# DerekGloudemans/3D-playground

Hardware: AMD Instinct MI355X
Metric: training images/sec at 1920x1080, ResNet-50 3D-RetinaNet (higher is better)
Workload: dtype f32; 1 GPU; resnet50 directional 3D-RetinaNet, 1920x1080 synthetic frames, batch 8 per GPU, 10 GT boxes/image, fp32, fwd+loss+bwd+clip+Adam (BASELINE configs[1]); global_batch=8, parallelism=dp1

## Files before the change

3d-playground_amd/csrc/conv_wino.hip:

```cpp
#include "common.h"
#include "mfma_split.h"

__device__ __forceinline__ float4 f4(float s) { return make_float4(s, s, s, s); }
typedef float nt_f4 __attribute__((ext_vector_type(4)));
__device__ __forceinline__ float4 ld_stream(const float *p) {
    const nt_f4 v = __builtin_nontemporal_load(reinterpret_cast<const nt_f4 *>(p));
    return make_float4(v.x, v.y, v.z, v.w);
}
__device__ __forceinline__ void st_stream(float *p, float4 v) { *reinterpret_cast<float4 *>(p) = v; }
__device__ __forceinline__ float4 operator+(float4 a, float4 b) { return make_float4(a.x + b.x, a.y + b.y, a.z + b.z, a.w + b.w); }
__device__ __forceinline__ float4 operator-(float4 a, float4 b) { return make_float4(a.x - b.x, a.y - b.y, a.z - b.z, a.w - b.w); }
__device__ __forceinline__ float4 operator*(float s, float4 a) { return make_float4(s * a.x, s * a.y, s * a.z, s * a.w); }

__device__ __forceinline__ void bt6(const float4 d[6], float4 o[6]) {
    o[0] = 4.f * d[0] - 5.f * d[2] + d[4];
    o[1] = d[3] + d[4] - 4.f * (d[1] + d[2]);
    o[2] = 4.f * (d[1] - d[2]) - d[3] + d[4];
    o[3] = 2.f * (d[3] - d[1]) - d[2] + d[4];
    o[4] = 2.f * (d[1] - d[3]) - d[2] + d[4];
    o[5] = 4.f * d[1] - 5.f * d[3] + d[5];
}
__device__ __forceinline__ void at6(const float4 m[6], float4 o[4]) {
    const float4 s12 = m[1] + m[2], d12 = m[1] - m[2], s34 = m[3] + m[4], d34 = m[3] - m[4];
    o[0] = m[0] + s12 + s34;
    o[1] = d12 + 2.f * d34;
    o[2] = s12 + 4.f * s34;
    o[3] = d12 + 8.f * d34 + m[5];
}


struct WinoProblem { int N, H, W, TH, TW; };
struct WinoTable {
    int n;
    int64_t tile_end[RN_MAX_GROUP];
    WinoProblem p[RN_MAX_GROUP];
    const float *src[RN_MAX_GROUP];
    float *dst[RN_MAX_GROUP];
    const float *add[RN_MAX_GROUP];
    const float *mask[RN_MAX_GROUP];
    unsigned *sign[RN_MAX_GROUP];
    unsigned *amax[RN_MAX_GROUP];
};

#define WINO_GAIN_BT 7
#define WINO_GAIN_A 8
__device__ __forceinline__ void wino_tensor_word(const WinoTable &g, unsigned *tensor_amax, int gain) {
    if (tensor_amax == nullptr || blockIdx.x != 0 || threadIdx.x >= 64) return;
    int e = 0;
#pragma unroll
    for (int i = 0; i < RN_MAX_GROUP; ++i)
        if (i < g.n && g.amax[i] != nullptr) { const int ei = rn_amax_exp_all(g.amax[i], g.p[i].N); e = ei > e ? ei : e; }
    if (threadIdx.x == 0) atomicMax(tensor_amax, rn_amax_word_of_exp(e, gain));
}
__device__ __forceinline__ int wino_locate(const WinoTable &g, int64_t gt, int64_t &local) {
    int q = 0;
#pragma unroll
    for (int i = 0; i < RN_MAX_GROUP - 1; ++i) q += (i + 1 < g.n && gt >= g.tile_end[i]) ? 1 : 0;
    int64_t first = 0;
#pragma unroll
    for (int i = 1; i < RN_MAX_GROUP; ++i)
        if (q == i) first = g.tile_end[i - 1];
    local = gt - first;
    return q;
}

#define WINO_SELECT(q, g, pr, EXTRA)                          \
    WinoProblem pr = g.p[0];                                   \
    _Pragma("unroll") for (int i_ = 1; i_ < RN_MAX_GROUP; ++i_) \
        if (q == i_) { pr = g.p[i_]; EXTRA }

__global__ __launch_bounds__(256) void wino_in_kernel(const WinoTable g, float *__restrict__ V, int C, int64_t t0, int64_t Tpad,
                                                      unsigned *__restrict__ row_amax, unsigned *__restrict__ tensor_amax) {
    wino_tensor_word(g, tensor_amax, WINO_GAIN_BT);
    const int cq = C >> 2;
    const int64_t id = (int64_t)xcd_remap(blockIdx.x, gridDim.x) * 256 + threadIdx.x;
    const int64_t gt_raw = id / cq, t_last = g.tile_end[g.n - 1];
    const int64_t gt = gt_raw < t_last ? gt_raw : t_last - 1;
    const int c4 = (int)(id - gt_raw * cq) * 4;
    int64_t tile;
    const int q = wino_locate(g, gt, tile);
    const float *x = g.src[0];
    const unsigned *xw = g.amax[0];
    WINO_SELECT(q, g, pr, x = g.src[i_]; xw = g.amax[i_];)
    const int H = pr.H, W = pr.W, TW = pr.TW;
    const int n = (int)(tile / (pr.TH * TW));
    const int r = (int)(tile - (int64_t)n * pr.TH * TW);
    const int th = r / TW, tw = r - th * TW;
    const int h0 = 4 * th - 1, w0 = 4 * tw - 1;
    const float *xb = x + (int64_t)n * H * W * C + c4;
    if (row_amax != nullptr) {
        const int e_img = rn_amax_exp_lanes(xw != nullptr ? reinterpret_cast<const unsigned char *>(xw) + (int64_t)n * RN_AMAX_BYTES : nullptr);
        if (gt_raw < t_last && c4 == 0) row_amax[t0 + gt] = rn_amax_word_of_exp(e_img, WINO_GAIN_BT);
    }
    if (gt_raw >= t_last) return;
    float4 t[6][6];
#pragma unroll
    for (int j = 0; j < 6; ++j) {
        float4 d[6], o[6];
        const int w = w0 + j;
#pragma unroll
        for (int i = 0; i < 6; ++i) {
            const int h = h0 + i;
#ifdef RN_WINO_ABL
            const bool ok = (unsigned)h < (unsigned)H && (unsigned)w < (unsigned)W && i >= 1 && i <= 4 && j >= 1 && j <= 4;
#else
            const bool ok = (unsigned)h < (unsigned)H && (unsigned)w < (unsigned)W;
#endif
            d[i] = ok ? *reinterpret_cast<const float4 *>(xb + ((int64_t)h * W + w) * C) : f4(0.f);
        }
        bt6(d, o);
#pragma unroll
        for (int i = 0; i < 6; ++i) t[i][j] = o[i];
    }
    float *vb = V + (t0 + gt) * C + c4;
#pragma unroll
    for (int i = 0; i < 6; ++i) {
        float4 o[6];
        bt6(t[i], o);
#pragma unroll
        for (int j = 0; j < 6; ++j) st_stream(vb + (int64_t)(i * 6 + j) * Tpad * C, o[j]);
    }
}

template <bool PBITS, bool PADD>
__global__ __launch_bounds__(256, 2) void wino_out_kernel(const WinoTable g, const float *__restrict__ M, int Cout, int64_t t0,
                                                       int64_t Tpad, const float *__restrict__ scale,
                                                       const float *__restrict__ shift, int mask_mode, int act, int64_t y_bs) {
    const int cq = Cout >> 2;
    const int64_t id = (int64_t)blockIdx.x * 256 + threadIdx.x;
    const int64_t gt = id / cq;
    float am = 0.f;
    unsigned *yam = nullptr;
    int n_img = 0;
    bool live = false;
    do {
    if (gt >= g.tile_end[g.n - 1]) break;
    live = true;
    const int c4 = (int)(id - gt * cq) * 4;
    int64_t tile;
    const int q = wino_locate(g, gt, tile);
    float *y = g.dst[0];
    const float *add = g.add[0], *mask = g.mask[0];
    unsigned *sign = g.sign[0];
    yam = g.amax[0];
    WINO_SELECT(q, g, pr, y = g.dst[i_]; add = g.add[i_]; mask = g.mask[i_]; sign = g.sign[i_]; yam = g.amax[i_];)
    n_img = (int)(tile / (pr.TH * pr.TW));
    const bool mbits = (mask_mode & RN_MASK_BITS) != 0;
    mask_mode &= 3;
    const int H = pr.H, W = pr.W, TW = pr.TW;
    const int n = (int)(tile / (pr.TH * TW));
    const int r = (int)(tile - (int64_t)n * pr.TH * TW);
    const int th = r / TW, tw = r - th * TW;
    const float *mb = M + (t0 + gt) * Cout + c4;
    float4 t[4][6];
#pragma unroll
    for (int j = 0; j < 6; ++j) {
        float4 m[6], o[4];
#pragma unroll
        for (int i = 0; i < 6; ++i) m[i] = ld_stream(mb + (int64_t)(i * 6 + j) * Tpad * Cout);
        at6(m, o);
#pragma unroll
        for (int i = 0; i < 4; ++i) t[i][j] = o[i];
    }
    float4 sc = f4(1.f), sh = f4(0.f);
    if (scale) sc = *reinterpret_cast<const float4 *>(scale + c4);
    if (shift) sh = *reinterpret_cast<const float4 *>(shift + c4);
    const int64_t ybs = y_bs ? y_bs : (int64_t)H * W * Cout;
#pragma unroll
    for (int i = 0; i < 4; ++i) {
        float4 o[4];
        at6(t[i], o);
        const int oh = 4 * th + i;
        if (oh >= H) break;
        unsigned mkw[4];
        float4 adv[4];
        if constexpr (PBITS || PADD) {
#pragma unroll
            for (int j = 0; j < 4; ++j) {
                const int owc = 4 * tw + j < W ? 4 * tw + j : W - 1;
                const int64_t off = (((int64_t)n * H + oh) * W + owc) * Cout + c4;
                if constexpr (PBITS) mkw[j] = reinterpret_cast<const unsigned *>(mask)[off >> 5] >> ((unsigned)off & 28u);
                if constexpr (PADD) adv[j] = *reinterpret_cast<const float4 *>(add + off);
            }
        }
#pragma unroll
        for (int j = 0; j < 4; ++j) {
            const int ow = 4 * tw + j;
            if (ow >= W) break;
            const int64_t off = (((int64_t)n * H + oh) * W + ow) * Cout + c4;
            const int64_t yoff = (int64_t)n * ybs + ((int64_t)oh * W + ow) * Cout + c4;
            float v[4] = {sc.x * o[j].x + sh.x, sc.y * o[j].y + sh.y, sc.z * o[j].z + sh.z, sc.w * o[j].w + sh.w};
            float mk[4] = {1.f, 1.f, 1.f, 1.f}, ad[4] = {0.f, 0.f, 0.f, 0.f};
            if constexpr (PBITS) {
                const unsigned nb = mkw[j];
                mk[0] = (nb & 1u) ? 1.f : 0.f; mk[1] = (nb & 2u) ? 1.f : 0.f; mk[2] = (nb & 4u) ? 1.f : 0.f; mk[3] = (nb & 8u) ? 1.f : 0.f;
            } else if (mask_mode != 0) { const float4 q4 = rn_mask_load4(mask, off, mbits); mk[0] = q4.x; mk[1] = q4.y; mk[2] = q4.z; mk[3] = q4.w; }
            if constexpr (PADD) { const float4 q4 = adv[j]; ad[0] = q4.x; ad[1] = q4.y; ad[2] = q4.z; ad[3] = q4.w; }
            else if (add) { const float4 q4 = *reinterpret_cast<const float4 *>(add + off); ad[0] = q4.x; ad[1] = q4.y; ad[2] = q4.z; ad[3] = q4.w; }
#pragma unroll
            for (int k = 0; k < 4; ++k) {
                float u = v[k];
                if (mask_mode == 1) u = mk[k] > 0.f ? u : 0.f;
                u += ad[k];
                if (act == 1) u = fmaxf(u, 0.f);
                else if (act == 2) u = 1.0f / (1.0f + expf(-u));
                if (mask_mode == 2) u = mk[k] > 0.f ? u : 0.f;
                v[k] = u;
            }
            *reinterpret_cast<float4 *>(y + yoff) = make_float4(v[0], v[1], v[2], v[3]);
            if (sign != nullptr) rn_sign_store(sign, off, v[0], v[1], v[2], v[3]);
            am = fmaxf(fmaxf(am, fmaxf(fabsf(v[0]), fabsf(v[1]))), fmaxf(fabsf(v[2]), fabsf(v[3])));
        }
    }
    } while (0);
    if (live) rn_amax_note(yam, n_img, am);
}

__global__ void wino_weight_kernel(const float *__restrict__ w, float *__restrict__ U, int Cout, int Cin, int mode,
                                   const float *__restrict__ scale, int rows, int Kpad) {
    const int64_t id = (int64_t)blockIdx.x * 256 + threadIdx.x;
    if (id >= (int64_t)rows * Kpad) return;
    const int row = (int)(id / Kpad), k = (int)(id - (int64_t)row * Kpad);
    const int kdim = mode == 0 ? Cin : Cout;
    float g[3][3];
#pragma unroll
    for (int r = 0; r < 3; ++r)
#pragma unroll
        for (int s = 0; s < 3; ++s) {
            float v = 0.f;
            if (k < kdim) {
                if (mode == 0) v = w[(((int64_t)row * Cin + k) * 3 + r) * 3 + s];
                else v = w[(((int64_t)k * Cin + row) * 3 + (2 - r)) * 3 + (2 - s)] * (scale ? scale[k] : 1.f);
            }
            g[r][s] = v;
        }
    float t[6][3];
#pragma unroll
    for (int s = 0; s < 3; ++s) {
        const float a = g[0][s], b = g[1][s], c = g[2][s];
        t[0][s] = a * (1.f / 4.f);
        t[1][s] = -(a + b + c) * (1.f / 6.f);
        t[2][s] = (b - a - c) * (1.f / 6.f);
        t[3][s] = a * (1.f / 24.f) + b * (1.f / 12.f) + c * (1.f / 6.f);
        t[4][s] = a * (1.f / 24.f) - b * (1.f / 12.f) + c * (1.f / 6.f);
        t[5][s] = c;
    }
#pragma unroll
    for (int i = 0; i < 6; ++i) {
        const float a = t[i][0], b = t[i][1], c = t[i][2];
        const float o[6] = {a * (1.f / 4.f), -(a + b + c) * (1.f / 6.f), (b - a - c) * (1.f / 6.f),
                            a * (1.f / 24.f) + b * (1.f / 12.f) + c * (1.f / 6.f),
                            a * (1.f / 24.f) - b * (1.f / 12.f) + c * (1.f / 6.f), c};
#pragma unroll
        for (int j = 0; j < 6; ++j) U[((int64_t)(i * 6 + j) * rows + row) * Kpad + k] = o[j];
    }
}

__device__ __forceinline__ void a6(const float4 v[4], float4 o[6]) {
    const float4 s02 = v[0] + v[2], s13 = v[1] + v[3];
    o[0] = v[0];
    o[1] = s02 + s13;
    o[2] = s02 - s13;
    const float4 e = v[0] + 4.f * v[2], f = 2.f * v[1] + 8.f * v[3];
    o[3] = e + f;
    o[4] = e - f;
    o[5] = v[3];
}

__global__ __launch_bounds__(256) void wino_dy_kernel(const WinoTable g, float *__restrict__ Z, int C, int64_t t0, int64_t Tpad,
                                                      unsigned *__restrict__ tensor_amax) {
    wino_tensor_word(g, tensor_amax, WINO_GAIN_A);
    const int cq = C >> 2;
    const int64_t id = (int64_t)blockIdx.x * 256 + threadIdx.x;
    const int64_t gt = id / cq;
    if (gt >= g.tile_end[g.n - 1]) return;
    const int c4 = (int)(id - gt * cq) * 4;
    int64_t tile;
    const int q = wino_locate(g, gt, tile);
    const float *dy = g.src[0];
    WINO_SELECT(q, g, pr, dy = g.src[i_];)
    const int H = pr.H, W = pr.W, TW = pr.TW;
    const int n = (int)(tile / (pr.TH * TW));
    const int r = (int)(tile - (int64_t)n * pr.TH * TW);
    const int th = r / TW, tw = r - th * TW;
    const float *yb = dy + (int64_t)n * H * W * C + c4;
    float4 t[6][4];
#pragma unroll
    for (int j = 0; j < 4; ++j) {
        float4 v[4], o[6];
        const int w = 4 * tw + j;
#pragma unroll
        for (int i = 0; i < 4; ++i) {
            const int h = 4 * th + i;
            v[i] = (h < H && w < W) ? *reinterpret_cast<const float4 *>(yb + ((int64_t)h * W + w) * C) : f4(0.f);
        }
        a6(v, o);
#pragma unroll
        for (int a = 0; a < 6; ++a) t[a][j] = o[a];
    }
    float *zb = Z + (t0 + gt) * C + c4;
#pragma unroll
    for (int a = 0; a < 6; ++a) {
        float4 o[6];
        a6(t[a], o);
#pragma unroll
        for (int b = 0; b < 6; ++b) st_stream(zb + (int64_t)(a * 6 + b) * Tpad * C, o[b]);
    }
}

__global__ __launch_bounds__(256) void wino_in_both_kernel(const WinoTable g, float *__restrict__ V, float *__restrict__ Z, int C,
                                                           int64_t t0, int64_t Tpad, unsigned *__restrict__ v_row_amax,
                                                           unsigned *__restrict__ z_tensor_amax) {
    wino_tensor_word(g, z_tensor_amax, WINO_GAIN_A);
    const int cq = C >> 2;
    const int64_t id = (int64_t)xcd_remap(blockIdx.x, gridDim.x) * 256 + threadIdx.x;
    const int64_t gt_raw = id / cq, t_last = g.tile_end[g.n - 1];
    const int64_t gt = gt_raw < t_last ? gt_raw : t_last - 1;
    const int c4 = (int)(id - gt_raw * cq) * 4;
    int64_t tile;
    const int q = wino_locate(g, gt, tile);
    const float *x = g.src[0];
    const unsigned *xw = g.amax[0];
    WINO_SELECT(q, g, pr, x = g.src[i_]; xw = g.amax[i_];)
    const int H = pr.H, W = pr.W, TW = pr.TW;
    const int n = (int)(tile / (pr.TH * TW));
    const int r = (int)(tile - (int64_t)n * pr.TH * TW);
    const int th = r / TW, tw = r - th * TW;
    const int h0 = 4 * th - 1, w0 = 4 * tw - 1;
    const float *xb = x + (int64_t)n * H * W * C + c4;
    if (v_row_amax != nullptr) {
        const int e_img = rn_amax_exp_lanes(xw != nullptr ? reinterpret_cast<const unsigned char *>(xw) + (int64_t)n * RN_AMAX_BYTES : nullptr);
        if (gt_raw < t_last && c4 == 0) v_row_amax[t0 + gt] = rn_amax_word_of_exp(e_img, WINO_GAIN_BT);
    }
    if (gt_raw >= t_last) return;
    float4 t[6][6];
    float4 tz[6][4];
#pragma unroll
    for (int j = 0; j < 6; ++j) {
        float4 d[6], o[6];
        const int w = w0 + j;
#pragma unroll
        for (int i = 0; i < 6; ++i) {
            const int h = h0 + i;
            const bool ok = (unsigned)h < (unsigned)H && (unsigned)w < (unsigned)W;
            d[i] = ok ? *reinterpret_cast<const float4 *>(xb + ((int64_t)h * W + w) * C) : f4(0.f);
        }
        bt6(d, o);
#pragma unroll
        for (int i = 0; i < 6; ++i) t[i][j] = o[i];
        if (j >= 1 && j <= 4) {
            float4 oz[6];
            a6(d + 1, oz);
#pragma unroll
            for (int a = 0; a < 6; ++a) tz[a][j - 1] = oz[a];
        }
    }
    float *zb = Z + (t0 + gt) * C + c4;
#pragma unroll
    for (int a = 0; a < 6; ++a) {
        float4 o[6];
        a6(tz[a], o);
#pragma unroll
        for (int b = 0; b < 6; ++b) st_stream(zb + (int64_t)(a * 6 + b) * Tpad * C, o[b]);
    }
    float *vb = V + (t0 + gt) * C + c4;
#pragma unroll
    for (int i = 0; i < 6; ++i) {
        float4 o[6];
        bt6(t[i], o);
#pragma unroll
        for (int j = 0; j < 6; ++j) st_stream(vb + (int64_t)(i * 6 + j) * Tpad * C, o[j]);
    }
}

__global__ void wino_dw_kernel(const float *__restrict__ dU, float *__restrict__ dw, int Cout, int Cin, int Ku, int Kpad) {
    const int64_t id = (int64_t)blockIdx.x * 256 + threadIdx.x;
    if (id >= (int64_t)Cout * Cin) return;
    const int co = (int)(id / Cin), ci = (int)(id - (int64_t)co * Cin);
    const float *u = dU + (int64_t)co * Ku + ci;
    const int64_t ps = (int64_t)Cout * Ku;
    float t[3][6];
#pragma unroll
    for (int j = 0; j < 6; ++j) {
        float v[6];
#pragma unroll
        for (int i = 0; i < 6; ++i) v[i] = u[(i * 6 + j) * ps];
        t[0][j] = v[0] * (1.f / 4.f) - (v[1] + v[2]) * (1.f / 6.f) + (v[3] + v[4]) * (1.f / 24.f);
        t[1][j] = (v[2] - v[1]) * (1.f / 6.f) + (v[3] - v[4]) * (1.f / 12.f);
        t[2][j] = (v[3] + v[4] - v[1] - v[2]) * (1.f / 6.f) + v[5];
    }
    float *o = dw + (int64_t)co * Kpad + ci;
#pragma unroll
    for (int r = 0; r < 3; ++r) {
        const float *v = t[r];
        o[(r * 3 + 0) * Cin] += v[0] * (1.f / 4.f) - (v[1] + v[2]) * (1.f / 6.f) + (v[3] + v[4]) * (1.f / 24.f);
        o[(r * 3 + 1) * Cin] += (v[2] - v[1]) * (1.f / 6.f) + (v[3] - v[4]) * (1.f / 12.f);
        o[(r * 3 + 2) * Cin] += (v[3] + v[4] - v[1] - v[2]) * (1.f / 6.f) + v[5];
    }
}

static int wino_table(const rn_wino_group *g, WinoTable &t) {
    if (!g || g->n < 1 || g->n > RN_MAX_GROUP) return RN_EINVAL;
    t.n = g->n;
    int64_t end = 0;
    for (int i = 0; i < RN_MAX_GROUP; ++i) {
        const int k = i < g->n ? i : g->n - 1;
        if (g->N[k] <= 0 || g->H[k] <= 0 || g->W[k] <= 0) return RN_EINVAL;
        t.p[i].N = g->N[k]; t.p[i].H = g->H[k]; t.p[i].W = g->W[k];
        t.p[i].TH = (g->H[k] + 3) / 4; t.p[i].TW = (g->W[k] + 3) / 4;
        if (i < g->n) end += (int64_t)g->N[k] * t.p[i].TH * t.p[i].TW;
        t.tile_end[i] = end;
        t.src[i] = g->src[k]; t.dst[i] = g->dst[k]; t.add[i] = g->add[k]; t.mask[i] = g->mask[k];
        t.sign[i] = reinterpret_cast<unsigned *>(g->sign[k]);
        t.amax[i] = reinterpret_cast<unsigned *>(g->amax[k]);
    }
    return RN_OK;
}

extern "C" int rn_wino_input_group(const rn_wino_group *g, float *V, int C, int64_t tile_offset, int64_t Tpad, int dy_form,
                                   void *row_amax, void *tensor_amax, void *stream) {
    WinoTable t;
    const int rc = wino_table(g, t);
    if (rc) return rc;
    if (C <= 0 || (C & 3) || tile_offset < 0 || tile_offset + t.tile_end[t.n - 1] > Tpad) return RN_EINVAL;
    for (int i = 0; i < t.n; ++i)
        if (!t.src[i]) return RN_EINVAL;
    const dim3 grid(rn_blocks(t.tile_end[t.n - 1] * (C >> 2), 256));
    if (dy_form && row_amax != nullptr) return RN_EINVAL;
    if (dy_form) hipLaunchKernelGGL(wino_dy_kernel, grid, dim3(256), 0, (hipStream_t)stream, t, V, C, tile_offset, Tpad,
                                    reinterpret_cast<unsigned *>(tensor_amax));
    else hipLaunchKernelGGL(wino_in_kernel, grid, dim3(256), 0, (hipStream_t)stream, t, V, C, tile_offset, Tpad,
                            reinterpret_cast<unsigned *>(row_amax), reinterpret_cast<unsigned *>(tensor_amax));
    RN_LAUNCH_CHECK();
    return RN_OK;
}

extern "C" int rn_wino_input_both_group(const rn_wino_group *g, float *V, float *Z, int C, int64_t tile_offset, int64_t Tpad,
                                        void *v_row_amax, void *z_tensor_amax, void *stream) {
    WinoTable t;
    const int rc = wino_table(g, t);
    if (rc) return rc;
    if (!V || !Z || C <= 0 || (C & 3) || tile_offset < 0 || tile_offset + t.tile_end[t.n - 1] > Tpad) return RN_EINVAL;
    for (int i = 0; i < t.n; ++i)
        if (!t.src[i]) return RN_EINVAL;
    hipLaunchKernelGGL(wino_in_both_kernel, dim3(rn_blocks(t.tile_end[t.n - 1] * (C >> 2), 256)), dim3(256), 0, (hipStream_t)stream, t,
                       V, Z, C, tile_offset, Tpad, reinterpret_cast<unsigned *>(v_row_amax), reinterpret_cast<unsigned *>(z_tensor_amax));
    RN_LAUNCH_CHECK();
    return RN_OK;
}

extern "C" int rn_wino_output_group(const rn_wino_group *g, const float *M, int Cout, int64_t tile_offset, int64_t Tpad,
                                    const float *scale, const float *shift, int mask_mode, int act, int64_t y_batch_stride,
                                    void *stream) {
    WinoTable t;
    const int rc = wino_table(g, t);
    if (rc) return rc;
    if (Cout <= 0 || (Cout & 3) || tile_offset < 0 || tile_offset + t.tile_end[t.n - 1] > Tpad) return RN_EINVAL;
    if (mask_mode < 0 || (mask_mode & ~(3 | RN_MASK_BITS)) || (mask_mode & 3) == 3 || mask_mode == RN_MASK_BITS) return RN_EINVAL;
    if (act < 0 || act > 2 || y_batch_stride < 0 || (y_batch_stride & 3)) return RN_EINVAL;
    for (int i = 0; i < t.n; ++i) {
        if (!t.dst[i] || (mask_mode != 0) != (t.mask[i] != nullptr)) return RN_EINVAL;
        if (((mask_mode & RN_MASK_BITS) || t.sign[i]) && (Cout & 31)) return RN_EINVAL;
        if (y_batch_stride && y_batch_stride < (int64_t)t.p[i].H * t.p[i].W * Cout) return RN_EINVAL;
    }
    const bool pbits = (mask_mode & RN_MASK_BITS) != 0;
    bool padd = true;
    for (int i = 0; i < t.n; ++i) padd = padd && t.add[i] != nullptr;
    const dim3 grid(rn_blocks(t.tile_end[t.n - 1] * (Cout >> 2), 256));
#define RN_WINO_OUT(B, A) hipLaunchKernelGGL((wino_out_kernel<B, A>), grid, dim3(256), 0, (hipStream_t)stream, t, M, Cout, tile_offset, Tpad, \
                                             scale, shift, mask_mode, act, y_batch_stride)
    if (pbits && padd) RN_WINO_OUT(true, true);
    else if (pbits) RN_WINO_OUT(true, false);
    else if (padd) RN_WINO_OUT(false, true);
    else RN_WINO_OUT(false, false);
#undef RN_WINO_OUT
    RN_LAUNCH_CHECK();
    return RN_OK;
}

static rn_wino_group wino_single(const float *src, float *dst, const float *add, const float *mask, int N, int H, int W) {
    rn_wino_group g = {};
    g.n = 1; g.N[0] = N; g.H[0] = H; g.W[0] = W; g.src[0] = src; g.dst[0] = dst; g.add[0] = add; g.mask[0] = mask;
    return g;
}
extern "C" int rn_wino_input(const float *x, float *V, int N, int H, int W, int C, int64_t tile_offset, int64_t Tpad,
                             void *stream) {
    const rn_wino_group g = wino_single(x, nullptr, nullptr, nullptr, N, H, W);
    return rn_wino_input_group(&g, V, C, tile_offset, Tpad, 0, nullptr, nullptr, stream);
}
extern "C" int rn_wino_dy(const float *dy, float *Z, int N, int H, int W, int C, int64_t tile_offset, int64_t Tpad, void *stream) {
    const rn_wino_group g = wino_single(dy, nullptr, nullptr, nullptr, N, H, W);
    return rn_wino_input_group(&g, Z, C, tile_offset, Tpad, 1, nullptr, nullptr, stream);
}
extern "C" int rn_wino_output(const float *M, float *y, int N, int H, int W, int Cout, int64_t tile_offset, int64_t Tpad,
                              const float *scale, const float *shift, const float *add, const float *mask, int mask_mode,
                              int act, int64_t y_batch_stride, void *stream) {
    const rn_wino_group g = wino_single(nullptr, y, add, mask, N, H, W);
    return rn_wino_output_group(&g, M, Cout, tile_offset, Tpad, scale, shift, mask_mode, act, y_batch_stride, stream);
}

extern "C" int rn_wino_weights(const float *w, float *U, int Cout, int Cin, int mode, const float *scale, void *stream) {
    if (Cout <= 0 || Cin <= 0 || mode < 0 || mode > 1) return RN_EINVAL;
    const int rows = mode == 0 ? Cout : Cin;
    const int Kpad = ((mode == 0 ? Cin : Cout) + 31) / 32 * 32;
    hipLaunchKernelGGL(wino_weight_kernel, dim3(rn_blocks((int64_t)rows * Kpad, 256)), dim3(256), 0, (hipStream_t)stream, w, U,
                       Cout, Cin, mode, scale, rows, Kpad);
    RN_LAUNCH_CHECK();
    return RN_OK;
}

extern "C" int rn_wino_dw(const float *dU, float *dw, int Cout, int Cin, void *stream) {
    if (Cout <= 0 || Cin <= 0) return RN_EINVAL;
    const int Ku = (Cin + 31) / 32 * 32, Kpad = (9 * Cin + 31) / 32 * 32;
    hipLaunchKernelGGL(wino_dw_kernel, dim3(rn_blocks((int64_t)Cout * Cin, 256)), dim3(256), 0, (hipStream_t)stream, dU, dw, Cout,
                       Cin, Ku, Kpad);
    RN_LAUNCH_CHECK();
    return RN_OK;
}
```

Measured before the change: 127.0 images/sec.

## Add LDS-staged Winograd output transform for small tile counts

Adds a Winograd output-transform kernel that stages the 36 transform planes into LDS with global_load_lds DMA before computing the inverse transform. It uses one channel per thread with 256-thread blocks by default, which gives more parallelism on layers with few tiles. It is chosen when the tile count is below a threshold that an environment variable can override, and the original float4 kernel handles larger layers. The aim is more coalesced reads and better latency hiding for small feature maps, at the cost of scalar stores and extra LDS traffic.

```diff
diff --git a/3d-playground_amd/csrc/conv_wino.hip b/3d-playground_amd/csrc/conv_wino.hip
--- a/3d-playground_amd/csrc/conv_wino.hip
+++ b/3d-playground_amd/csrc/conv_wino.hip
@@ -216,6 +216,181 @@
     if (live) rn_amax_note(yam, n_img, am);
 }
 
+#ifndef RN_WINO_OUT_VEC
+#define RN_WINO_OUT_VEC 1
+#endif
+#ifndef RN_WINO_OUT_STAGED_BELOW
+#define RN_WINO_OUT_STAGED_BELOW 1536
+#endif
+template <int V> struct wvec { float a[V]; };
+template <int V> __device__ __forceinline__ wvec<V> operator+(wvec<V> x, wvec<V> y) {
+    wvec<V> r;
+#pragma unroll
+    for (int k = 0; k < V; ++k) r.a[k] = x.a[k] + y.a[k];
+    return r;
+}
+template <int V> __device__ __forceinline__ wvec<V> operator-(wvec<V> x, wvec<V> y) {
+    wvec<V> r;
+#pragma unroll
+    for (int k = 0; k < V; ++k) r.a[k] = x.a[k] - y.a[k];
+    return r;
+}
+template <int V> __device__ __forceinline__ wvec<V> operator*(float s, wvec<V> x) {
+    wvec<V> r;
+#pragma unroll
+    for (int k = 0; k < V; ++k) r.a[k] = s * x.a[k];
+    return r;
+}
+template <int V> __device__ __forceinline__ wvec<V> ldv(const float *p) {
+    wvec<V> r;
+    if constexpr (V == 4) { const float4 q = *reinterpret_cast<const float4 *>(p); r.a[0] = q.x; r.a[1] = q.y; r.a[2] = q.z; r.a[3] = q.w; }
+    else if constexpr (V == 2) { const float2 q = *reinterpret_cast<const float2 *>(p); r.a[0] = q.x; r.a[1] = q.y; }
+    else r.a[0] = *p;
+    return r;
+}
+template <int V> __device__ __forceinline__ void at6v(const wvec<V> m[6], wvec<V> o[4]) {
+    const wvec<V> s12 = m[1] + m[2], d12 = m[1] - m[2], s34 = m[3] + m[4], d34 = m[3] - m[4];
+    o[0] = m[0] + s12 + s34;
+    o[1] = d12 + 2.f * d34;
+    o[2] = s12 + 4.f * s34;
+    o[3] = d12 + 8.f * d34 + m[5];
+}
+
+template <bool PBITS, bool PADD, int V>
+__global__ __launch_bounds__(V == 4 ? 64 : 256) void wino_out_staged_kernel(const WinoTable g, const float *__restrict__ M, int Cout,
+                                                                            int64_t t0, int64_t Tpad, const float *__restrict__ scale,
+                                                                            const float *__restrict__ shift, int mask_mode, int act,
+                                                                            int64_t y_bs) {
+    static_assert(V == 1 || V == 4, "channels per thread");
+    constexpr int WAVES = V == 4 ? 1 : 4;
+    constexpr int SPAN = 64 * V;
+    constexpr int LPS = SPAN / 4, PPI = 64 / LPS, NI = 36 / PPI;
+    __shared__ __attribute__((aligned(16))) float strip[WAVES][36 * SPAN];
+    const int lane = threadIdx.x & 63, wave = __builtin_amdgcn_readfirstlane(threadIdx.x >> 6);
+    const int cg = Cout / V;
+    const int64_t total = g.tile_end[g.n - 1] * cg;
+    const int64_t e0 = ((int64_t)blockIdx.x * WAVES + wave) * 64;
+    if (e0 >= total) return;
+    {
+        int64_t f = e0 * V + (lane % LPS) * 4;
+        f = f < total * V - 4 ? f : total * V - 4;
+        const float *src = M + t0 * Cout + f + (int64_t)(lane / LPS) * Tpad * Cout;
+        const int64_t istep = (int64_t)PPI * Tpad * Cout;
+#pragma unroll
+        for (int i = 0; i < NI; ++i)
+            __builtin_amdgcn_global_load_lds((const __attribute__((address_space(1))) void *)(src + i * istep),
+                                             (__attribute__((address_space(3))) void *)&strip[wave][i * 256], 16, 0,
+                                             2);
+    }
+    const int64_t e = e0 + lane;
+    float am = 0.f;
+    unsigned *yam = nullptr;
+    int n_img = 0;
+    const bool live = e < total;
+    const bool small = total <= 0x7fffffff;
+    const int64_t gt = !live ? g.tile_end[g.n - 1] - 1 : small ? (int64_t)((unsigned)e / (unsigned)cg) : e / cg;
+    const int c4 = live ? (int)(e - gt * cg) * V : 0;
+    int64_t tile;
+    const int q = wino_locate(g, gt, tile);
+    float *y = g.dst[0];
+    const float *add = g.add[0], *mask = g.mask[0];
+    unsigned *sign = g.sign[0];
+    yam = g.amax[0];
+    WINO_SELECT(q, g, pr, y = g.dst[i_]; add = g.add[i_]; mask = g.mask[i_]; sign = g.sign[i_]; yam = g.amax[i_];)
+    mask_mode &= 3;
+    const int H = pr.H, W = pr.W, TW = pr.TW;
+    const int n = small ? (int)((unsigned)tile / (unsigned)(pr.TH * TW)) : (int)(tile / (pr.TH * TW));
+    n_img = n;
+    const int r = (int)(tile - (int64_t)n * pr.TH * TW);
+    const int th = r / TW, tw = r - th * TW;
+    wvec<V> sc, sh;
+#pragma unroll
+    for (int k = 0; k < V; ++k) { sc.a[k] = 1.f; sh.a[k] = 0.f; }
+    if (scale) sc = ldv<V>(scale + c4);
+    if (shift) sh = ldv<V>(shift + c4);
+    const int64_t ybs = y_bs ? y_bs : (int64_t)H * W * Cout;
+    rn_wait_dma();
+    if (live) {
+    const float *ms = &strip[wave][lane * V];
+    wvec<V> t[4][6];
+#pragma unroll
+    for (int j = 0; j < 6; ++j) {
+        wvec<V> m[6], o[4];
+#pragma unroll
+        for (int i = 0; i < 6; ++i) m[i] = ldv<V>(ms + (i * 6 + j) * SPAN);
+        at6v<V>(m, o);
+#pragma unroll
+        for (int i = 0; i < 4; ++i) t[i][j] = o[i];
+    }
+#pragma unroll
+    for (int i = 0; i < 4; ++i) {
+        wvec<V> o[4];
+        at6v<V>(t[i], o);
+        const int oh = 4 * th + i;
+        if (oh >= H) break;
+        unsigned mkw[4];
+        wvec<V> adv[4];
+        if constexpr (PBITS || PADD) {
+#pragma unroll
+            for (int j = 0; j < 4; ++j) {
+                const int owc = 4 * tw + j < W ? 4 * tw + j : W - 1;
+                const int64_t off = (((int64_t)n * H + oh) * W + owc) * Cout + c4;
+                if constexpr (PBITS) mkw[j] = reinterpret_cast<const unsigned *>(mask)[off >> 5] >> ((unsigned)off & (32u - V));
+                if constexpr (PADD) adv[j] = ldv<V>(add + off);
+            }
+        }
+#pragma unroll
+        for (int j = 0; j < 4; ++j) {
+            const int ow = 4 * tw + j;
+            if (ow >= W) break;
+            const int64_t off = (((int64_t)n * H + oh) * W + ow) * Cout + c4;
+            const int64_t yoff = (int64_t)n * ybs + ((int64_t)oh * W + ow) * Cout + c4;
+            float v[V], mk[V], ad[V];
+#pragma unroll
+            for (int k = 0; k < V; ++k) { v[k] = sc.a[k] * o[j].a[k] + sh.a[k]; mk[k] = 1.f; ad[k] = 0.f; }
+            if constexpr (PBITS) {
+#pragma unroll
+                for (int k = 0; k < V; ++k) mk[k] = (mkw[j] & (1u << k)) ? 1.f : 0.f;
+            } else if (mask_mode != 0) {
+                const wvec<V> q4 = ldv<V>(mask + off);
+#pragma unroll
+                for (int k = 0; k < V; ++k) mk[k] = q4.a[k];
+            }
+            if constexpr (PADD) {
+#pragma unroll
+                for (int k = 0; k < V; ++k) ad[k] = adv[j].a[k];
+            } else if (add) {
+                const wvec<V> q4 = ldv<V>(add + off);
+#pragma unroll
+                for (int k = 0; k < V; ++k) ad[k] = q4.a[k];
+            }
+#pragma unroll
+            for (int k = 0; k < V; ++k) {
+                float u = v[k];
+                if (mask_mode == 1) u = mk[k] > 0.f ? u : 0.f;
+                u += ad[k];
+                if (act == 1) u = fmaxf(u, 0.f);
+                else if (act == 2) u = 1.0f / (1.0f + expf(-u));
+                if (mask_mode == 2) u = mk[k] > 0.f ? u : 0.f;
+                v[k] = u;
+                am = fmaxf(am, fabsf(u));
+            }
+            if constexpr (V == 4) {
+                *reinterpret_cast<float4 *>(y + yoff) = make_float4(v[0], v[1], v[2], v[3]);
+                if (sign != nullptr) rn_sign_store(sign, off, v[0], v[1], v[2], v[3]);
+            } else {
+                y[yoff] = v[0];
+                if (sign != nullptr) {
+                    const unsigned long long b = __ballot(v[0] > 0.f);
+                    if ((lane & 31) == 0) sign[off >> 5] = (unsigned)(b >> (lane & 32));
+                }
+            }
+        }
+    }
+    rn_amax_note(yam, n_img, am);
+    }
+}
+
 __global__ void wino_weight_kernel(const float *__restrict__ w, float *__restrict__ U, int Cout, int Cin, int mode,
                                    const float *__restrict__ scale, int rows, int Kpad) {
     const int64_t id = (int64_t)blockIdx.x * 256 + threadIdx.x;
@@ -466,7 +641,22 @@
     const bool pbits = (mask_mode & RN_MASK_BITS) != 0;
     bool padd = true;
     for (int i = 0; i < t.n; ++i) padd = padd && t.add[i] != nullptr;
-    const dim3 grid(rn_blocks(t.tile_end[t.n - 1] * (Cout >> 2), 256));
+    static const int64_t staged_below = [] { const char *e = getenv("RN_WINO_OUT_STAGED_BELOW_TILES"); return e ? atoll(e) : (int64_t)RN_WINO_OUT_STAGED_BELOW; }();
+    const int64_t tiles = t.tile_end[t.n - 1];
+    if (tiles < staged_below) {
+        constexpr int V = RN_WINO_OUT_VEC, WG = V == 4 ? 64 : 256;
+        const dim3 grid(rn_blocks(tiles * (Cout / V), WG));
+#define RN_WINO_OUT(B, A) hipLaunchKernelGGL((wino_out_staged_kernel<B, A, V>), grid, dim3(WG), 0, (hipStream_t)stream, t, M, Cout, tile_offset, \
+                                             Tpad, scale, shift, mask_mode, act, y_batch_stride)
+        if (pbits && padd) RN_WINO_OUT(true, true);
+        else if (pbits) RN_WINO_OUT(true, false);
+        else if (padd) RN_WINO_OUT(false, true);
+        else RN_WINO_OUT(false, false);
+#undef RN_WINO_OUT
+        RN_LAUNCH_CHECK();
+        return RN_OK;
+    }
+    const dim3 grid(rn_blocks(tiles * (Cout >> 2), 256));
 #define RN_WINO_OUT(B, A) hipLaunchKernelGGL((wino_out_kernel<B, A>), grid, dim3(256), 0, (hipStream_t)stream, t, M, Cout, tile_offset, Tpad, \
                                              scale, shift, mask_mode, act, y_batch_stride)
     if (pbits && padd) RN_WINO_OUT(true, true);
```

Measured after the change: 127.2 images/sec (median of 5 runs). About the same (+0.2%).
